# wgurecky/bipymc

Hardware: AMD Instinct MI355X
Metric: chain-updates/sec (higher is better)
Workload: dtype f64

## Files before the change

### bipymc_amd/csrc/kernels.h

```cpp
#pragma once
#ifndef __HIPCC_RTC__
#include <hip/hip_runtime.h>
#include <stdint.h>
#endif

#include "philox.h"

#ifdef BPM_STAMPS
#define BPM_STAMP(i)                                                                          \
    do {                                                                                      \
        __builtin_amdgcn_sched_barrier(0);                                                    \
        unsigned long long _t;                                                                \
        asm volatile("s_memtime %0\n\ts_waitcnt lgkmcnt(0)" : "=s"(_t)::"memory");            \
        __builtin_amdgcn_sched_barrier(0);                                                    \
        bpm_stamp[i] = _t;                                                                    \
    } while (0)
#else
#define BPM_STAMP(i) do { } while (0)
#endif

#if defined(__HIP_DEVICE_COMPILE__) && !defined(__gfx942__) && !defined(__gfx950__)
#error "kernels.h: the ticket hand-overs rely on gfx942 / gfx950 memory behaviour (vmcnt counts stores; agent-scope atomics bypass the L2s): use __ATOMIC_RELEASE / __ATOMIC_ACQUIRE tickets on other targets"
#endif

// ... 114 lines not shown
    uint32_t upd_off, n_upd, pool_off, M;
    uint32_t mode;
    uint32_t n_items;
    uint32_t algo;
    uint32_t P, n_cr;
    double* cr_part1;
    const double* cr_fold_part;
    const double* cr_fold_tot;
    double* cr_fold_out;
    uint32_t cr_fold_nb;
    uint32_t cr_chunk0, cr_n1;
    uint32_t adapt_on;
    uint32_t cr_gate;
    uint32_t hist_len;
    double gamma_scale, gamma_demc, epsilon, u_epsilon, p_snooker;
#ifdef BPM_LEAN_LAST
    uint32_t lean, pad_lean;
#endif
};

#ifdef BPM_TEST_HOOKS
__host__ __device__ __forceinline__ int32_t* trace_i32_of(const PhaseArgs& a) { return a.trace_i32; }
__host__ __device__ __forceinline__ double* trace_f64_of(const PhaseArgs& a) { return a.trace_f64; }
__host__ __device__ __forceinline__ uint8_t* trace_mask_of(const PhaseArgs& a) { return a.trace_mask; }
__host__ __device__ __forceinline__ void trace_set(PhaseArgs& a, int32_t* i, double* f, uint8_t* m) { a.trace_i32 = i; a.trace_f64 = f; a.trace_mask = m; }
#else
__host__ __device__ constexpr int32_t* trace_i32_of(const PhaseArgs&) { return nullptr; }
__host__ __device__ constexpr double* trace_f64_of(const PhaseArgs&) { return nullptr; }
__host__ __device__ constexpr uint8_t* trace_mask_of(const PhaseArgs&) { return nullptr; }
__host__ __device__ __forceinline__ void trace_set(PhaseArgs&, int32_t*, double*, uint8_t*) {}
#endif

template <int CTRL>
__device__ __forceinline__ double dpp_f64(double v) {
    const int lo = __builtin_amdgcn_update_dpp(0, __double2loint(v), CTRL, 0xF, 0xF, false);
    const int hi = __builtin_amdgcn_update_dpp(0, __double2hiint(v), CTRL, 0xF, 0xF, false);
    return __hiloint2double(hi, lo);
}
__device__ __forceinline__ double readlane_f64(double v, int lane) {
    return __hiloint2double(__builtin_amdgcn_readlane(__double2hiint(v), lane),
                            __builtin_amdgcn_readlane(__double2loint(v), lane));
}
template <int LPC>
__device__ __forceinline__ double gsum(double v) {
    static_assert(LPC == 1 || LPC == 4 || LPC == 16 || LPC == 32 || LPC == 64, "subgroup sizes");
    if (LPC >= 4) {
        v += dpp_f64<0xB1>(v);
        v += dpp_f64<0x4E>(v);
    }
    if (LPC >= 16) {
        v += dpp_f64<0x141>(v);
        v += dpp_f64<0x140>(v);
    }
    if (LPC == 32) v += __shfl_xor(v, 16);
    if (LPC == 64) v = (readlane_f64(v, 0) + readlane_f64(v, 16)) + (readlane_f64(v, 32) + readlane_f64(v, 48));
    return v;
}
template <int LPC>
__device__ __forceinline__ void gsum2(double& v, double& w) {
    static_assert(LPC == 1 || LPC == 4 || LPC == 16 || LPC == 32 || LPC == 64, "subgroup sizes");
    if (LPC >= 4) {
        const double v1 = dpp_f64<0xB1>(v), w1 = dpp_f64<0xB1>(w);
        v += v1; w += w1;
        const double v2 = dpp_f64<0x4E>(v), w2 = dpp_f64<0x4E>(w);
        v += v2; w += w2;
    }
    if (LPC >= 16) {
        const double v3 = dpp_f64<0x141>(v), w3 = dpp_f64<0x141>(w);
        v += v3; w += w3;
        const double v4 = dpp_f64<0x140>(v), w4 = dpp_f64<0x140>(w);
        v += v4; w += w4;
    }
    if (LPC == 32) { const double vs = __shfl_xor(v, 16), ws = __shfl_xor(w, 16); v += vs; w += ws; }
    if (LPC == 64) {
        const double va = readlane_f64(v, 0) + readlane_f64(v, 16), wa = readlane_f64(w, 0) + readlane_f64(w, 16);
        const double vb = readlane_f64(v, 32) + readlane_f64(v, 48), wb = readlane_f64(w, 32) + readlane_f64(w, 48);
        v = va + vb; w = wa + wb;
    }
}
template <int LPC>
__device__ __forceinline__ int gsum_i(int v) {
    if (LPC >= 4) {
        v += __builtin_amdgcn_update_dpp(0, v, 0xB1, 0xF, 0xF, false);
        v += __builtin_amdgcn_update_dpp(0, v, 0x4E, 0xF, 0xF, false);
    }
    if (LPC >= 16) {
        v += __builtin_amdgcn_update_dpp(0, v, 0x141, 0xF, 0xF, false);
        v += __builtin_amdgcn_update_dpp(0, v, 0x140, 0xF, 0xF, false);
    }
    if (LPC == 32) v += __shfl_xor(v, 16);
    if (LPC == 64)
        v = (__builtin_amdgcn_readlane(v, 0) + __builtin_amdgcn_readlane(v, 16)) +
            (__builtin_amdgcn_readlane(v, 32) + __builtin_amdgcn_readlane(v, 48));
    return v;
}

constexpr uint32_t CR_FINAL_MAX = 512;
__host__ __device__ inline uint32_t cr_chunks_of(uint32_t n_half, uint32_t g1) { return (n_half + g1 - 1u) / g1; }
struct CrTotals { double p[MAX_CR], d[MAX_CR], n[MAX_CR]; };
__device__ __forceinline__ void cr_finalize(bool any, uint32_t n_cr, CrTotals& T) {
    if (!any) return;
    uint32_t nz = 0;
#pragma unroll
    for (int m = 0; m < MAX_CR; ++m) nz += (m < (int)n_cr && T.n[m] != 0.0) ? 1u : 0u;
    if (nz == n_cr) {
#pragma unroll
        for (int m = 0; m < MAX_CR; ++m) if (m < (int)n_cr) T.p[m] = T.d[m] / T.n[m];
    }
    double sum = 0.0;
#pragma unroll
    for (int m = 0; m < MAX_CR; ++m) if (m < (int)n_cr) sum += T.p[m];
#pragma unroll
    for (int m = 0; m < MAX_CR; ++m) if (m < (int)n_cr) T.p[m] = T.p[m] / sum;
}
template <int ROUNDS>
__device__ __forceinline__ double cr_array_sum(const double* arr, uint32_t nb) {
    const uint32_t lane = threadIdx.x & (WAVE - 1);
    double v[ROUNDS];
#pragma unroll
    for (int r = 0; r < ROUNDS; ++r) {
        const uint32_t b = (uint32_t)r * WAVE + lane;
        const double x = arr[b < nb ? b : nb - 1u];
        v[r] = b < nb ? x : 0.0;
    }
    double s = 0.0;
#pragma unroll
// ... 224 lines not shown
__device__ __forceinline__ void store_row_sys(double* row, int q, uint32_t ld, const double* v) {
#pragma unroll
    for (int u = 0; u < DPL / 2; ++u) {
        const uint32_t pi = (uint32_t)(q + u * LPC);
        if (2 * pi < ld) {
            __hip_atomic_store(row + 2 * pi, v[2 * u], __ATOMIC_RELAXED, __HIP_MEMORY_SCOPE_SYSTEM);
            __hip_atomic_store(row + 2 * pi + 1, v[2 * u + 1], __ATOMIC_RELAXED, __HIP_MEMORY_SCOPE_SYSTEM);
        }
    }
}

template <int LPC, int DPL>
__device__ __forceinline__ void store_row_stream(double* row, int q, uint32_t ld, const double* v) {
#pragma unroll
    for (int u = 0; u < DPL / 2; ++u) {
        const uint32_t pi = (uint32_t)(q + u * LPC);
        if (2 * pi < ld) {
            bpm_d2v t = {v[2 * u], v[2 * u + 1]};
            __builtin_nontemporal_store(t, reinterpret_cast<bpm_d2v*>(row) + pi);
        }
    }
}

__device__ __forceinline__ void box_muller_pair_f32(uint32_t w1, uint32_t w2, double& n0, double& n1) {
    const float u1 = ((float)w1 + 1.0f) * 2.3283064365386963e-10f;
    const float u2 = (float)w2 * 2.3283064365386963e-10f;
    const float r = __builtin_amdgcn_sqrtf(-2.0f * 0.6931471805599453f * __builtin_amdgcn_logf(u1));
    n0 = (double)(r * __builtin_amdgcn_cosf(u2));
    n1 = (double)(r * __builtin_amdgcn_sinf(u2));
}

template <int K>
__device__ __forceinline__ uint32_t quad_bcast(uint32_t v) {
    return (uint32_t)__builtin_amdgcn_update_dpp(0, (int)v, K * 0x55, 0xF, 0xF, false);
}

template <int LPC, int NPART_CT>
struct Partners {
    uint32_t r[NPART_CT > 0 ? NPART_CT : 1];
    const uint32_t* lds;
    __device__ __forceinline__ uint32_t get(int i) const { return NPART_CT > 0 ? r[i] : lds[i]; }
};

__device__ __forceinline__ uint32_t partner_pos(const PhaseArgs& a, uint32_t c, uint32_t idx, uint32_t n_pair_idx) {
    if (idx < n_pair_idx) {
        const uint32_t p = idx >> 1;
        const u32x4 wb = chain_block(a.seed, c, a.t, SLOT_PAIR0 + (p >> 1));
        uint32_t ia, ib;
        distinct_pair((p & 1) ? wb.z : wb.x, (p & 1) ? wb.w : wb.y, a.M, ia, ib);
        uint32_t pos = (idx & 1) ? ib : ia;
        if (a.mode == 2) pos += (pos >= c) ? 1u : 0u;
        return pos;
    }
    const u32x4 ws = chain_block(a.seed, c, a.t, SLOT_SNK);
    uint32_t iz, i1, i2;
    distinct_three(ws.x, ws.y, ws.z, a.M, iz, i1, i2);
    const uint32_t s = idx - n_pair_idx;
    return s == 0 ? iz : (s == 1 ? i1 : i2);
}

__device__ __forceinline__ uint32_t pos_to_chain(const PhaseArgs& a, uint32_t pos) {
#if defined(BPM_TEST_HOOKS) && defined(BPM_FAKE_NO_PARTNER_HOP)
    return pos;
#else
    return a.perm_tab ? a.perm_tab[pos] : perm_fwd(pos, a.pk);
#endif
}
__device__ __forceinline__ uint32_t own_pos_to_chain(const PhaseArgs& a, uint32_t pos) {
#if defined(BPM_TEST_HOOKS) && defined(BPM_FAKE_NO_OWN_HOP)
    return pos;
#else
    return a.perm_tab ? a.perm_tab[pos] : perm_fwd(pos, a.pk);
#endif
}
__device__ __forceinline__ uint32_t chain_to_pos(const PhaseArgs& a, uint32_t c) {
    return a.inv_tab ? a.inv_tab[c] : perm_inv(c, a.pk);
}

template <int DPL, int NPX>
struct PlanFront {
    uint32_t rec[PLAN_WORDS];
    double x[DPL], ra[NPX][DPL], rb[NPX][DPL];
    double ll_cur, pcr[3], gl[DPL];
    uint32_t acc_prev;
};
typedef uint32_t bpm_u32x16 __attribute__((ext_vector_type(16)));
__device__ __forceinline__ bpm_u32x16 plan_record(const uint32_t* recp) {
    return *reinterpret_cast<const bpm_u32x16*>(__builtin_assume_aligned(recp, 4 * PLAN_WORDS));
}
template <int DPL, int NP>
__device__ __forceinline__ void plan_front(const Layout& L, const bpm_u32x16 rv, int q, PlanFront<DPL, (NP > 0 ? NP : 1)>& fr) {
    static_assert(PLAN_WORDS == 16 && DPL == 2, "one 64-byte record, one 16-byte load per lane and row");
#pragma unroll
    for (int i = 0; i < PLAN_WORDS; ++i) fr.rec[i] = rv[i];
    load_row_all<WAVE, DPL>(row_ptr(L, fr.rec[0]), q, L.ld, fr.x);
#pragma unroll
    for (int p = 0; p < NP; ++p) {
        load_row_all<WAVE, DPL>(row_ptr(L, fr.rec[5 + 2 * p]), q, L.ld, fr.ra[p]);
        load_row_all<WAVE, DPL>(row_ptr(L, fr.rec[5 + 2 * p + 1]), q, L.ld, fr.rb[p]);
    }
    __builtin_amdgcn_sched_barrier(0);
}

struct NoEarly { template <class W> __device__ __forceinline__ void operator()(W&) const {} };
struct PcrGiven { bool on = false; double p[MAX_CR]; };
template <int ALGO, int LPC, int DPL, int NP, int LOAD_LL = 1 , class EARLY = NoEarly, bool FRONT = false>
__device__ __forceinline__ void make_proposal(const PhaseArgs& a, uint32_t c, bool active, int q, int cw,
                                              uint32_t* s_part, Work<DPL>& wk, const uint32_t* rec = nullptr,
                                              unsigned long long* bpm_stamp = nullptr, EARLY early = EARLY(), const PcrGiven pcr_ovr = PcrGiven(),
                                              const PlanFront<DPL, (NP > 0 ? NP : 1)>* fr = nullptr) {
    static_assert(!FRONT || (LPC == WAVE && DPL == 2), "the planned front serves one wavefront per chain with one coordinate pair per lane");
    constexpr bool DREAM = ALGO == ALGO_DREAM;
    constexpr bool FAST = (NP > 0) && (LPC == 1);
    constexpr bool SNK_DIRECT = (LPC == 1);
    const uint32_t dim = a.L.dim, ld = a.L.ld;
    const uint32_t P = NP > 0 ? (uint32_t)NP : a.P;
    if constexpr (FRONT) {
        const bool in_row = 2u * (uint32_t)q < ld;
#pragma unroll
        for (int s = 0; s < DPL; ++s) wk.x[s] = in_row ? fr->x[s] : 0.0;
    } else
    load_row<LPC, DPL>(row_ptr(a.L, c), q, ld, wk.x);
    wk.ll_cur = 0.0;
    wk.acc_prev = 0u;
    if (!a.replay) {
#if defined(BPM_TEST_HOOKS) && defined(BPM_FAKE_NO_LL)
        if (LPC < WAVE) wk.ll_cur = wk.x[0] * 1e-300; else
#endif
        if constexpr (FRONT) wk.ll_cur = fr->ll_cur; else
        if (LOAD_LL == 1 || (LOAD_LL == 2 && !a.lean)) wk.ll_cur = a.ll[c - a.lo];
        if constexpr (FRONT) wk.acc_prev = fr->acc_prev; else
        if (LPC == WAVE) wk.acc_prev = a.acc_count[c - a.lo];
// ... 11 lines not shown
    double gtab[DPL];
    if (DREAM && LPC == WAVE) {
#pragma unroll
        for (int u = 0; u < DPL; ++u) {
            const uint32_t gi = (uint32_t)(q + u * WAVE);
            const double gl = FRONT ? fr->gl[u] : a.gamma_tab[gi <= dim ? gi : dim];
            gtab[u] = gi <= dim ? gl : 0.0;
        }
    }
    double gt_lane = 0.0;
    if (DREAM && LPC * DPL < WAVE) {
        const uint32_t wl = (uint32_t)threadIdx.x & (uint32_t)(WAVE - 1);
        gt_lane = a.gamma_tab[wl <= dim ? wl : dim];
    }
    const bool snk_possible = !DREAM && a.p_snooker > 0.0 && a.M >= 3;
    const uint32_t npart = 2 * P + (snk_possible ? 3u : 0u);
    constexpr bool RL = (LPC == WAVE) && (NP > 0) && !FAST;
    const uint32_t npairs = (dim + 1u) >> 1;
    const bool merged = !FRONT && RL && DPL == 2 && (npairs + 2u * (uint32_t)NP + 1u <= (uint32_t)WAVE);
    u32x4 wpair[DPL / 2];
    u32x4 h0;
    constexpr bool QUAD = DREAM && LPC == 4 && DPL == 2 && NP == 3;
    constexpr bool REGS = FAST || RL || QUAD;
    Partners<LPC, REGS ? 2 * NP : 0> part;
    part.lds = s_part + cw * MAX_PARTNERS;
    const bool planned = FRONT || ((LPC == WAVE) && rec != nullptr);
    const bool dims_late = planned && RL && DPL == 2;
    if (FRONT) {
        h0.x = fr->rec[1]; h0.y = fr->rec[2]; h0.z = fr->rec[3]; h0.w = fr->rec[4];
#pragma unroll
        for (int i = 0; i < 2 * NP; ++i) part.r[i] = fr->rec[5 + i];
        if (!dims_late) {
#pragma unroll
            for (int u = 0; u < DPL / 2; ++u) wpair[u] = chain_block(a.seed, c, a.t, SLOT_DIM0 + (uint32_t)(q + u * LPC));
        }
    } else if (planned) {
        h0.x = rec[1]; h0.y = rec[2]; h0.z = rec[3]; h0.w = rec[4];
        if (FAST || RL) {
#pragma unroll
            for (int i = 0; i < 2 * NP; ++i) part.r[i] = rec[5 + i];
        }
        if (!dims_late) {
#pragma unroll
            for (int u = 0; u < DPL / 2; ++u) wpair[u] = chain_block(a.seed, c, a.t, SLOT_DIM0 + (uint32_t)(q + u * LPC));
        }
    } else if (merged) {
        const uint32_t uq = (uint32_t)q, hdr_lane = npairs + 2u * (uint32_t)NP;
        const uint32_t pidx = uq - npairs;
        const uint32_t slot = uq < npairs ? SLOT_DIM0 + uq : (uq < hdr_lane ? SLOT_PAIR0 + (pidx >> 2) : SLOT_HDR0);
        const u32x4 wb = chain_block(a.seed, c, a.t, slot);
        wpair[0] = wb;
        h0.x = (uint32_t)__builtin_amdgcn_readlane((int)wb.x, hdr_lane);
        h0.y = (uint32_t)__builtin_amdgcn_readlane((int)wb.y, hdr_lane);
        h0.z = (uint32_t)__builtin_amdgcn_readlane((int)wb.z, hdr_lane);
        h0.w = (uint32_t)__builtin_amdgcn_readlane((int)wb.w, hdr_lane);
        BPM_STAMP(2);
        uint32_t mine = 0;
        if (uq >= npairs && uq < hdr_lane) {
            const uint32_t p = pidx >> 1;
            uint32_t ia, ib;
            distinct_pair((p & 1) ? wb.z : wb.x, (p & 1) ? wb.w : wb.y, a.M, ia, ib);
            uint32_t pos = (pidx & 1) ? ib : ia;
            if (a.mode == 2) pos += (pos >= c) ? 1u : 0u;
            mine = pos_to_chain(a, a.pool_off + pos);
        }
#pragma unroll
        for (int i = 0; i < 2 * NP; ++i) part.r[i] = (uint32_t)__builtin_amdgcn_readlane((int)mine, npairs + i);
    } else if (QUAD) {
        wpair[0] = chain_block(a.seed, c, a.t, SLOT_DIM0 + (uint32_t)q);
        const u32x4 wb = chain_block(a.seed, c, a.t, q == 1 ? SLOT_PAIR0 : (q == 2 ? SLOT_PAIR0 + 1u : SLOT_HDR0));
        h0.x = quad_bcast<0>(wb.x); h0.y = quad_bcast<0>(wb.y); h0.z = quad_bcast<0>(wb.z); h0.w = quad_bcast<0>(wb.w);
        uint32_t i0 = 0, i1 = 0, i2 = 0, i3 = 0;
        if (q == 1 || q == 2) {
            uint32_t ia, ib;
            distinct_pair(wb.x, wb.y, a.M, ia, ib);
            i0 = pos_to_chain(a, a.pool_off + ia); i1 = pos_to_chain(a, a.pool_off + ib);
            if (q == 1) {
                distinct_pair(wb.z, wb.w, a.M, ia, ib);
                i2 = pos_to_chain(a, a.pool_off + ia); i3 = pos_to_chain(a, a.pool_off + ib);
            }
        }
        part.r[0] = quad_bcast<1>(i0); part.r[1] = quad_bcast<1>(i1); part.r[2] = quad_bcast<1>(i2); part.r[3] = quad_bcast<1>(i3);
        part.r[4] = quad_bcast<2>(i0); part.r[5] = quad_bcast<2>(i1);
    } else {
        h0 = chain_block(a.seed, c, a.t, SLOT_HDR0);
#pragma unroll
        for (int u = 0; u < DPL / 2; ++u) wpair[u] = chain_block(a.seed, c, a.t, SLOT_DIM0 + (uint32_t)(q + u * LPC));
        if (FAST) {
#pragma unroll
            for (int i = 0; i < 2 * NP; ++i) part.r[i] = pos_to_chain(a, a.pool_off + partner_pos(a, c, (uint32_t)i, 2u * NP));
        }
        if (RL) {
            uint32_t mine = 0;
            if (q < 2 * NP) mine = pos_to_chain(a, a.pool_off + partner_pos(a, c, (uint32_t)q, 2u * NP));
#pragma unroll
            for (int i = 0; i < 2 * NP; ++i) part.r[i] = (uint32_t)__builtin_amdgcn_readlane((int)mine, i);
        }
    }
    BPM_STAMP(3);
    wk.u_acc = u01_53(h0.z, h0.w);
    const double u_sel = (double)(h0.x >> 16) * 1.52587890625e-05;
    const double u_gam = (double)(h0.x & 0xFFFFu) * 1.52587890625e-05;
    uint32_t snk_id[3] = {0u, 0u, 0u};
    if (SNK_DIRECT && snk_possible && planned) {
        snk_id[0] = rec[5 + 2 * P]; snk_id[1] = rec[6 + 2 * P]; snk_id[2] = rec[7 + 2 * P];
    } else if (SNK_DIRECT && snk_possible && (u_sel < a.p_snooker || trace_i32_of(a) != nullptr)) {
        const u32x4 ws = chain_block(a.seed, c, a.t, SLOT_SNK);
        uint32_t iz, i1, i2;
        distinct_three(ws.x, ws.y, ws.z, a.M, iz, i1, i2);
        snk_id[0] = pos_to_chain(a, a.pool_off + iz);
        snk_id[1] = pos_to_chain(a, a.pool_off + i1);
        snk_id[2] = pos_to_chain(a, a.pool_off + i2);
    }
    if (!REGS || (snk_possible && !SNK_DIRECT)) {
#pragma unroll 1
        for (uint32_t idx = (uint32_t)q; idx < npart; idx += LPC)
            s_part[cw * MAX_PARTNERS + idx] = planned ? rec[5 + idx] : pos_to_chain(a, a.pool_off + partner_pos(a, c, idx, 2 * P));
        __builtin_amdgcn_fence(__ATOMIC_RELEASE, "wavefront");
        __builtin_amdgcn_wave_barrier();
        __builtin_amdgcn_fence(__ATOMIC_ACQUIRE, "wavefront");
    }

    constexpr int NPX = NP > 0 ? NP : 1;
    double ra[NPX][DPL], rb[NPX][DPL];
    if (FRONT && DREAM && NP > 0) {
#pragma unroll
        for (int p = 0; p < NP; ++p) {
#pragma unroll
            for (int s = 0; s < DPL; ++s) { ra[p][s] = fr->ra[p][s]; rb[p][s] = fr->rb[p][s]; }
        }
    } else if (DREAM && NP > 0) {
#pragma unroll
        for (int p = 0; p < NP; ++p) {
            if (LPC == WAVE) {
                load_row_all<LPC, DPL>(row_ptr(a.L, part.get(2 * p)), q, ld, ra[p]);
                load_row_all<LPC, DPL>(row_ptr(a.L, part.get(2 * p + 1)), q, ld, rb[p]);
            } else {
                load_row<LPC, DPL>(row_ptr(a.L, part.get(2 * p)), q, ld, ra[p]);
                load_row<LPC, DPL>(row_ptr(a.L, part.get(2 * p + 1)), q, ld, rb[p]);
            }
        }
    }
    if (!FRONT) BPM_STAMP(7);
    if (dims_late) wpair[0] = chain_block(a.seed, c, a.t, SLOT_DIM0 + (uint32_t)q);
    if (DREAM) early(wk);

    double eps_n[DPL], eps_u[DPL];
    uint32_t maskbits = 0;
    wk.cr_idx = -1; wk.d_prime = (int)dim; wk.jump = 0; wk.snk = 0; wk.delta = 0.0; wk.log_corr = 0.0;
    uint32_t thr = 65536u;
    if (DREAM) {
        const double uc = u_sel;
        double cum = 0.0;
        int idx = (int)a.n_cr - 1;
        bool found = false;
#pragma unroll
        for (int m = 0; m < MAX_CR; ++m) {
            if (m < (int)a.n_cr) {
                cum += pcr[m];
                if (!found && uc < cum) { idx = m; thr = a.thr[m]; found = true; }
            }
        }
        if (!found) {
#pragma unroll
            for (int m = 0; m < MAX_CR; ++m) if (m == (int)a.n_cr - 1) thr = a.thr[m];
        }
        wk.cr_idx = idx;
    }
    int cnt = 0;
#pragma unroll
    for (int u = 0; u < DPL / 2; ++u) {
        const uint32_t pi = (uint32_t)(q + u * LPC);
        const uint32_t j0 = 2u * pi;
        eps_n[2 * u] = 0.0; eps_n[2 * u + 1] = 0.0; eps_u[2 * u] = 0.0; eps_u[2 * u + 1] = 0.0;
        if (j0 < dim) {
            const u32x4 wj = wpair[u];
            const bool two = j0 + 1 < dim;
// ... 720 lines not shown
    const int cw = lane / LPC, q = lane % LPC;
    const uint32_t w = blockIdx.x * (block_for(LPC) / LPC) + cw;
    bool active = w < a.n_items;
    int32_t id = active ? a.ids_buf[w] : -1;
    active = active && id >= 0;
    if (LPC == WAVE && !active) return;
    const uint32_t c = active ? (uint32_t)id : a.lo;
    Work<DPL> wk;
    load_row<LPC, DPL>(row_ptr(a.L, c), q, a.L.ld, wk.x);
    load_row<LPC, DPL>(a.prop_buf + (uint64_t)(active ? w : 0u) * a.L.ld, q, a.L.ld, wk.p);
    wk.log_corr = active ? a.aux_buf[w] : 0.0;
    wk.ll_cur = a.ll[c - a.lo];
    wk.acc_prev = a.acc_count[c - a.lo];
    if (ALGO == ALGO_DREAM && a.adapt_on) {
        load_row<LPC, DPL>(a.w_mean + (uint32_t)((c - a.lo) * 2u * a.L.ld), q, a.L.ld, wk.w_mean);
        load_row<LPC, DPL>(a.w_m2 + (uint32_t)((c - a.lo) * 2u * a.L.ld), q, a.L.ld, wk.w_m2);
    }
    const double ll_prop = active ? a.aux_buf[a.L.n_local + w] : 0.0;
    const u32x4 h0 = chain_block(a.seed, c, a.t, SLOT_HDR0);
    wk.u_acc = u01_53(h0.z, h0.w);
    wk.delta = 0.0; wk.gamma = 0.0; wk.cr_idx = -1; wk.d_prime = 0; wk.jump = 0; wk.snk = 0; wk.maskbits = 0; wk.item = w; wk.pos_own = 0u;
    if (ALGO == ALGO_DREAM && active) {
        wk.delta = *delta_ptr(a.L, c);
        wk.cr_idx = (int)*cridx_ptr(a.L, c);
    }
    PhaseArgs b = a;
    if (ALGO == ALGO_DREAM) b.cr_gate = (wk.cr_idx >= 0) ? 1u : 0u;
    finish_update<ALGO, LPC, DPL>(b, c, active, q, wk, ll_prop);
}

constexpr int CR_L1_THREADS = 256;
template <int G1, int J>
__device__ __forceinline__ int cr_bcast_i(int v) {
    if (G1 == 4) return __builtin_amdgcn_update_dpp(0, v, J * 0x55, 0xF, 0xF, false);
    if (G1 == 16) return __builtin_amdgcn_update_dpp(0, v, 0x150 + J, 0xF, 0xF, false);
    return __builtin_amdgcn_readlane(v, J);
}
template <int G1, int J>
__device__ __forceinline__ void cr_l1_steps(int idx, double dl, int m0, double& sd0, double& sn0, double& sd1, double& sn1) {
    const int ij = cr_bcast_i<G1, J>(idx);
    const double dj = __hiloint2double(cr_bcast_i<G1, J>(__double2hiint(dl)), cr_bcast_i<G1, J>(__double2loint(dl)));
    cr_chunk_add(sd0, sn0, m0, ij, dj);
    if (G1 == 4) cr_chunk_add(sd1, sn1, m0 + 4, ij, dj);
    if constexpr (J + 1 < G1) cr_l1_steps<G1, J + 1>(idx, dl, m0, sd0, sn0, sd1, sn1);
}
template <int G1>
__global__ __launch_bounds__(CR_L1_THREADS) void cr_level1_kernel(Layout L, PermKey pk, const uint32_t* perm_tab, uint32_t N, uint32_t n_cr, uint32_t n1, double* part1) {
    const uint32_t t = blockIdx.x * CR_L1_THREADS + threadIdx.x;
    const uint32_t ch = t / G1, k = t % G1;
    const uint32_t n_first = (N + 1u) / 2u, c_first = cr_chunks_of(n_first, G1);
    const bool second = ch >= c_first;
    const uint32_t pos = second ? n_first + (ch - c_first) * G1 + k : ch * G1 + k;
    const bool valid = ch < n1 && pos < (second ? N : n_first);
    int idx = -1;
    double dl = 0.0;
    if (valid) {
        const uint32_t c = perm_tab ? perm_tab[pos] : perm_fwd(pos, pk);
        idx = (int)*cridx_ptr(L, c);
        dl = *delta_ptr(L, c);
    }
    static_assert(MAX_CR <= 8, "a chunk's lanes cover the CR values: lane k sums value k (and k + 4 when G1 == 4)");
    double sd0 = 0.0, sn0 = 0.0, sd1 = 0.0, sn1 = 0.0;
    cr_l1_steps<G1, 0>(idx, dl, (int)k, sd0, sn0, sd1, sn1);
    if (ch < n1) {
        if (k < n_cr) {
            __hip_atomic_store(&part1[(uint64_t)k * n1 + ch], sd0, __ATOMIC_RELAXED, __HIP_MEMORY_SCOPE_AGENT);
            __hip_atomic_store(&part1[(uint64_t)(MAX_CR + k) * n1 + ch], sn0, __ATOMIC_RELAXED, __HIP_MEMORY_SCOPE_AGENT);
        }
// ... 740 lines not shown
```

### bipymc_amd/csrc/kernels_wide.h

```cpp
#pragma once
#include "kernels.h"

namespace bpm {
inline namespace BPM_VARIANT_NS {

constexpr int WIDE_CP = 2;
constexpr int WIDE_CHUNK_PAIRS = WAVE * WIDE_CP;

template <int TARGET>
struct WideTarget {
    __device__ __forceinline__ void add(const double*, uint32_t, uint32_t, double, double) {}
    __device__ __forceinline__ double finish(const double*, uint32_t) { return 0.0; }
};
template <>
struct WideTarget<TARGET_GAUSS> {
    double s1 = 0.0, s2 = 0.0;
    __device__ __forceinline__ void add(const double* tp, uint32_t pi, uint32_t dim, double v0, double v1) {
        const uint32_t j0 = 2u * pi;
        if (j0 < dim) {
            const double2 is = *reinterpret_cast<const double2*>(tp + 4 + j0);
            const double z0 = v0 * is.x;
            s1 += z0; s2 += z0 * z0;
            if (j0 + 1u < dim) {
                const double z1 = v1 * is.y;
// ... 30 lines not shown
        return m + log(exp(c0 - m) + exp(c1 - m));
    }
};

__device__ __forceinline__ double2 wide_load2(const double* row, uint32_t pi, bool valid) {
    double2 t = make_double2(0.0, 0.0);
    if (valid) t = reinterpret_cast<const double2*>(row)[pi];
    return t;
}
__device__ __forceinline__ void wide_store2_stream(double* row, uint32_t pi, double v0, double v1) {
    bpm_d2v t = {v0, v1};
    __builtin_nontemporal_store(t, reinterpret_cast<bpm_d2v*>(row) + pi);
}
__device__ __forceinline__ void wide_store2_wt16(double* row, uint32_t pi, double v0, double v1) {
    bpm_d2v t = {v0, v1};
    bpm_d2v* p = reinterpret_cast<bpm_d2v*>(row) + pi;
    asm volatile("global_store_dwordx4 %0, %1, off sc1" ::"v"(p), "v"(t) : "memory");
}

struct WideUni {
    uint32_t dim, ld, P;
    uint32_t thr, forced;
    double gamma;
    double epsilon, u_epsilon;
    int snk;
    double gs;
};
template <int ALGO, int NP>
__device__ __forceinline__ void wide_pair_proposal(const PhaseArgs& a, const WideUni& U, uint32_t c, uint32_t pi, bool valid, double2 x, uint32_t mine,
                                                   double& p0, double& p1, uint32_t& mbits) {
    constexpr bool DREAM = ALGO == ALGO_DREAM;
    const uint32_t j0 = 2u * pi;
    const bool two = j0 + 1u < U.dim;
    const u32x4 wj = chain_block(a.seed, c, a.t, SLOT_DIM0 + pi);
    double en0 = 0.0, en1 = 0.0, eu0 = 0.0, eu1 = 0.0;
    mbits = 0u;
    if (valid) {
        if (U.epsilon > 0.0) {
            double n0, n1;
            box_muller_pair_f32(wj.z, wj.w, n0, n1);
            en0 = U.epsilon * n0;
            if (two) en1 = U.epsilon * n1;
        }
        if (DREAM) {
            if (U.u_epsilon > 0.0) {
                eu0 = -U.u_epsilon + (2.0 * U.u_epsilon) * (((double)(wj.y >> 16) + 0.5) * 1.52587890625e-05);
                if (two) eu1 = -U.u_epsilon + (2.0 * U.u_epsilon) * (((double)(wj.y & 0xFFFFu) + 0.5) * 1.52587890625e-05);
            }
            if ((wj.x >> 16) <= U.thr || j0 == U.forced) mbits |= 1u;
            if (two && ((wj.x & 0xFFFFu) <= U.thr || j0 + 1u == U.forced)) mbits |= 2u;
        }
    }
    if (DREAM) {
        double s0 = 0.0, s1 = 0.0;
        if (NP > 0) {
            double2 ra[NP > 0 ? NP : 1], rb[NP > 0 ? NP : 1];
#pragma unroll
            for (int p = 0; p < NP; ++p) {
                ra[p] = wide_load2(row_ptr(a.L, (uint32_t)__builtin_amdgcn_readlane((int)mine, 2 * p)), pi, valid);
                rb[p] = wide_load2(row_ptr(a.L, (uint32_t)__builtin_amdgcn_readlane((int)mine, 2 * p + 1)), pi, valid);
            }
            s0 = ra[0].x - rb[0].x; s1 = ra[0].y - rb[0].y;
#pragma unroll
            for (int p = 1; p < NP; ++p) { s0 = s0 + (ra[p].x - rb[p].x); s1 = s1 + (ra[p].y - rb[p].y); }
        } else {
#pragma unroll 1
            for (uint32_t p = 0; p < U.P; ++p) {
// ... 62 lines not shown
    uint32_t mine = 0;
    if (lane < npart) mine = pos_to_chain(a, a.pool_off + partner_pos(a, c, lane, 2u * U.P));
    double ll_cur = 0.0;
    uint32_t acc_prev = 0u;
    if (FUSED) { ll_cur = a.ll[li]; acc_prev = a.acc_count[li]; }
    const double u_sel = (double)(h0.x >> 16) * 1.52587890625e-05;
    const double u_gam = (double)(h0.x & 0xFFFFu) * 1.52587890625e-05;
    int cr_idx = -1, d_prime = (int)U.dim, jump = 0;
    if (DREAM) {
        double cum = 0.0;
        int idx = (int)a.n_cr - 1;
        bool found = false;
#pragma unroll
        for (int m = 0; m < MAX_CR; ++m) {
            if (m < (int)a.n_cr) {
                cum += a.cr_state[m];
                if (!found && u_sel < cum) { idx = m; found = true; }
            }
        }
        cr_idx = idx;
#pragma unroll
        for (int m = 0; m < MAX_CR; ++m) if (m == idx) U.thr = a.thr[m];
        int cnt = (int)U.dim;
        if (U.thr < 65536u) {
            cnt = 0;
#pragma unroll 1
            for (uint32_t k = 0; k < n_chunks; ++k) {
#pragma unroll
                for (int u = 0; u < WIDE_CP; ++u) {
                    const uint32_t pi = k * WIDE_CHUNK_PAIRS + (uint32_t)u * WAVE + lane;
                    const uint32_t j0 = 2u * pi;
                    bool b0 = false, b1 = false;
                    if (j0 < U.dim) {
                        const u32x4 wj = chain_block(a.seed, c, a.t, SLOT_DIM0 + pi);
                        b0 = (wj.x >> 16) <= U.thr;
                        b1 = (j0 + 1u < U.dim) && (wj.x & 0xFFFFu) <= U.thr;
                    }
                    cnt += (int)__popcll(__ballot(b0)) + (int)__popcll(__ballot(b1));
                }
            }
        }
        if (cnt == 0) { U.forced = mulhi32(h0.y, U.dim); cnt = 1; }
        d_prime = cnt;
        double gamma = a.gamma_tab[cnt];
        if (a.k % 5 == 0 && !(u_gam < 0.2)) { gamma = 1.0; jump = 1; }
        U.gamma = gamma;
    } else {
        double gamma = a.gamma_demc;
        if (a.mode != 2 && a.k % 10 == 0 && !(u_gam < 0.1)) { gamma = 1.0; jump = 1; }
        U.gamma = gamma;
    }
    double sn_n2 = 0.0;
    if (snk_possible && u_sel < a.p_snooker) {
        const double* zrow = row_ptr(a.L, (uint32_t)__builtin_amdgcn_readlane((int)mine, 2));
        const double* r1row = row_ptr(a.L, (uint32_t)__builtin_amdgcn_readlane((int)mine, 3));
        const double* r2row = row_ptr(a.L, (uint32_t)__builtin_amdgcn_readlane((int)mine, 4));
        double n2 = 0.0, dot = 0.0;
#pragma unroll 1
        for (uint32_t k = 0; k < n_chunks; ++k) {
#pragma unroll
            for (int u = 0; u < WIDE_CP; ++u) {
                const uint32_t pi = k * WIDE_CHUNK_PAIRS + (uint32_t)u * WAVE + lane;
                const bool valid = 2u * pi < U.dim;
                const double2 x = wide_load2(xrow, pi, valid), z = wide_load2(zrow, pi, valid), r1 = wide_load2(r1row, pi, valid), r2 = wide_load2(r2row, pi, valid);
                const double d0 = x.x - z.x, d1 = x.y - z.y;
                n2 += d0 * d0; dot += (r1.x - r2.x) * d0;
                n2 += d1 * d1; dot += (r1.y - r2.y) * d1;
// ... 247 lines not shown
```

### bipymc_amd/csrc/philox.h

```cpp
#pragma once
#ifndef __HIPCC_RTC__
#include <stdint.h>
#endif

#if defined(__HIPCC__)
#define BPM_HD __host__ __device__ __forceinline__
#else
#define BPM_HD inline
#endif

#ifndef BPM_VARIANT_NS
#ifdef BPM_TEST_HOOKS
#define BPM_VARIANT_NS hooks
#else
#define BPM_VARIANT_NS product
#endif
#endif
namespace bpm {
inline namespace BPM_VARIANT_NS {

constexpr int SLOT_BITS = 16;
constexpr uint32_t SLOT_HDR0 = 0;
constexpr uint32_t SLOT_PAIR0 = 2;
constexpr uint32_t SLOT_SNK = 7;
constexpr uint32_t SLOT_DIM0 = 8;
constexpr int MAX_PAIRS = 10;
constexpr uint64_t SUBSEQ_GLOBAL = 0xFFFFFFFFFFFFFFFFull;
constexpr uint32_t SLOT_G_FLIP = 0;
constexpr uint32_t SLOT_G_SHUF = 1;
constexpr uint64_t T_INIT = (1ull << 47) - 1;
constexpr int FEISTEL_ROUNDS = 6;

struct u32x4 {
    uint32_t x, y, z, w;
};

BPM_HD uint32_t mulhi32(uint32_t a, uint32_t b) {
#if defined(__HIP_DEVICE_COMPILE__)
    return __umulhi(a, b);
#else
    return (uint32_t)(((uint64_t)a * (uint64_t)b) >> 32);
#endif
}

BPM_HD u32x4 philox4x32_10(uint32_t c0, uint32_t c1, uint32_t c2, uint32_t c3, uint32_t k0, uint32_t k1) {
    constexpr uint32_t M0 = 0xD2511F53u, M1 = 0xCD9E8D57u, W0 = 0x9E3779B9u, W1 = 0xBB67AE85u;
#pragma unroll
    for (int r = 0; r < 10; ++r) {
        const uint64_t p0 = (uint64_t)M0 * (uint64_t)c0, p1 = (uint64_t)M1 * (uint64_t)c2;
        const uint32_t hi0 = (uint32_t)(p0 >> 32), lo0 = (uint32_t)p0;
        const uint32_t hi1 = (uint32_t)(p1 >> 32), lo1 = (uint32_t)p1;
        const uint32_t n0 = hi1 ^ c1 ^ k0, n2 = hi0 ^ c3 ^ k1;
        c0 = n0; c1 = lo1; c2 = n2; c3 = lo0;
        k0 += W0; k1 += W1;
    }
    return u32x4{c0, c1, c2, c3};
}

BPM_HD u32x4 philox_block(uint64_t seed, uint64_t subseq, uint64_t blk) {
    return philox4x32_10((uint32_t)blk, (uint32_t)(blk >> 32), (uint32_t)subseq, (uint32_t)(subseq >> 32),
                         (uint32_t)seed, (uint32_t)(seed >> 32));
}

BPM_HD u32x4 chain_block(uint64_t seed, uint64_t chain_id, uint64_t t, uint32_t slot) {
#if defined(BPM_TEST_HOOKS) && defined(BPM_FAKE_DRAWS) && defined(__HIP_DEVICE_COMPILE__)
    uint32_t x = (uint32_t)chain_id * 0x9e3779b9u + (uint32_t)t * 0x85ebca6bu + slot * 0xc2b2ae35u + (uint32_t)seed;
    x ^= x >> 15; x *= 0x2c1b3c6du; x ^= x >> 12;
    return u32x4{x, x * 0x297a2d39u, x ^ 0x5bd1e995u, x + 0x7f4a7c15u};
#else
    return philox_block(seed, chain_id, (t << SLOT_BITS) | (uint64_t)slot);
#endif
}

BPM_HD u32x4 global_block(uint64_t seed, uint64_t t, uint32_t slot) {
    return chain_block(seed, SUBSEQ_GLOBAL, t, slot);
}

BPM_HD double u01_32(uint32_t w) { return (double)w * 2.3283064365386963e-10; }

BPM_HD double u01_53(uint32_t hi, uint32_t lo) {
    return ((double)(hi >> 5) * 67108864.0 + (double)(lo >> 6)) * 1.1102230246251565e-16;
}

BPM_HD void distinct_pair(uint32_t wa, uint32_t wb, uint32_t m, uint32_t& ia, uint32_t& ib) {
    ia = mulhi32(wa, m);
    ib = mulhi32(wb, m - 1);
    ib += (ib >= ia) ? 1u : 0u;
}

BPM_HD void distinct_three(uint32_t wz, uint32_t w1, uint32_t w2, uint32_t m, uint32_t& iz, uint32_t& i1,
                           uint32_t& i2) {
    iz = mulhi32(wz, m);
    i1 = mulhi32(w1, m - 1);
    i1 += (i1 >= iz) ? 1u : 0u;
    const uint32_t lo = iz < i1 ? iz : i1, hi = iz < i1 ? i1 : iz;
    i2 = mulhi32(w2, m - 2);
    i2 += (i2 >= lo) ? 1u : 0u;
    i2 += (i2 >= hi) ? 1u : 0u;
}

BPM_HD uint32_t hash32(uint32_t x) {
    x ^= x >> 16; x *= 0x7FEB352Du; x ^= x >> 15; x *= 0x846CA68Bu; x ^= x >> 16;
    return x;
// ... 75 lines not shown
```

Measured before the change: 790.5 million.

## Use row-broadcast DPP reductions, bitop3 Philox XOR, and pinned scalar row bases

Several independent micro-optimisations land together. Full-wave sums now use DPP row_bcast15/31 followed by a single readlane instead of four readlanes, and DPP moves use mov_dpp with bound_ctrl. Philox rounds called from per-lane contexts use the gfx950 bitop3 three-input XOR to cut VALU instructions. The plan-front row loads precompute the base pointers, pin them in SGPRs through empty asm, and issue one clamped 16-byte global load per row in place of the generic load helper. The clamped index and changed reduction order can alter rounding and edge behaviour.

Measured after the change: 827.2 million, median of 6. +4.6%, better.

```diff
diff --git a/bipymc_amd/csrc/kernels.h b/bipymc_amd/csrc/kernels.h
--- a/bipymc_amd/csrc/kernels.h
+++ b/bipymc_amd/csrc/kernels.h
@@ -170,14 +170,24 @@
 #endif
 
 template <int CTRL>
+__device__ __forceinline__ int dpp_i32(int v) {
+    return __builtin_amdgcn_mov_dpp(v, CTRL, 0xF, 0xF, true);
+}
+template <int CTRL>
 __device__ __forceinline__ double dpp_f64(double v) {
-    const int lo = __builtin_amdgcn_update_dpp(0, __double2loint(v), CTRL, 0xF, 0xF, false);
-    const int hi = __builtin_amdgcn_update_dpp(0, __double2hiint(v), CTRL, 0xF, 0xF, false);
+    const int lo = dpp_i32<CTRL>(__double2loint(v));
+    const int hi = dpp_i32<CTRL>(__double2hiint(v));
     return __hiloint2double(hi, lo);
 }
 __device__ __forceinline__ double readlane_f64(double v, int lane) {
     return __hiloint2double(__builtin_amdgcn_readlane(__double2hiint(v), lane),
                             __builtin_amdgcn_readlane(__double2loint(v), lane));
+}
+constexpr int DPP_ROW_BCAST15 = 0x142, DPP_ROW_BCAST31 = 0x143;
+__device__ __forceinline__ double row_sums_step1_f64(double v) { return v + dpp_f64<DPP_ROW_BCAST15>(v); }
+__device__ __forceinline__ double row_sums_step2_f64(double v) { return v + dpp_f64<DPP_ROW_BCAST31>(v); }
+__device__ __forceinline__ double row_sums_f64(double v) {
+    return readlane_f64(row_sums_step2_f64(row_sums_step1_f64(v)), WAVE - 1);
 }
 template <int LPC>
 __device__ __forceinline__ double gsum(double v) {
@@ -191,7 +201,7 @@
         v += dpp_f64<0x140>(v);
     }
     if (LPC == 32) v += __shfl_xor(v, 16);
-    if (LPC == 64) v = (readlane_f64(v, 0) + readlane_f64(v, 16)) + (readlane_f64(v, 32) + readlane_f64(v, 48));
+    if (LPC == 64) v = row_sums_f64(v);
     return v;
 }
 template <int LPC>
@@ -211,25 +221,27 @@
     }
     if (LPC == 32) { const double vs = __shfl_xor(v, 16), ws = __shfl_xor(w, 16); v += vs; w += ws; }
     if (LPC == 64) {
-        const double va = readlane_f64(v, 0) + readlane_f64(v, 16), wa = readlane_f64(w, 0) + readlane_f64(w, 16);
-        const double vb = readlane_f64(v, 32) + readlane_f64(v, 48), wb = readlane_f64(w, 32) + readlane_f64(w, 48);
-        v = va + vb; w = wa + wb;
+        v = row_sums_step1_f64(v); w = row_sums_step1_f64(w);
+        v = row_sums_step2_f64(v); w = row_sums_step2_f64(w);
+        v = readlane_f64(v, WAVE - 1); w = readlane_f64(w, WAVE - 1);
     }
 }
 template <int LPC>
 __device__ __forceinline__ int gsum_i(int v) {
     if (LPC >= 4) {
-        v += __builtin_amdgcn_update_dpp(0, v, 0xB1, 0xF, 0xF, false);
-        v += __builtin_amdgcn_update_dpp(0, v, 0x4E, 0xF, 0xF, false);
+        v += dpp_i32<0xB1>(v);
+        v += dpp_i32<0x4E>(v);
     }
     if (LPC >= 16) {
-        v += __builtin_amdgcn_update_dpp(0, v, 0x141, 0xF, 0xF, false);
-        v += __builtin_amdgcn_update_dpp(0, v, 0x140, 0xF, 0xF, false);
+        v += dpp_i32<0x141>(v);
+        v += dpp_i32<0x140>(v);
     }
     if (LPC == 32) v += __shfl_xor(v, 16);
-    if (LPC == 64)
-        v = (__builtin_amdgcn_readlane(v, 0) + __builtin_amdgcn_readlane(v, 16)) +
-            (__builtin_amdgcn_readlane(v, 32) + __builtin_amdgcn_readlane(v, 48));
+    if (LPC == 64) {
+        v += dpp_i32<DPP_ROW_BCAST15>(v);
+        v += dpp_i32<DPP_ROW_BCAST31>(v);
+        v = __builtin_amdgcn_readlane(v, WAVE - 1);
+    }
     return v;
 }
 
@@ -520,7 +532,7 @@
 
 template <int K>
 __device__ __forceinline__ uint32_t quad_bcast(uint32_t v) {
-    return (uint32_t)__builtin_amdgcn_update_dpp(0, (int)v, K * 0x55, 0xF, 0xF, false);
+    return (uint32_t)dpp_i32<K * 0x55>((int)v);
 }
 
 template <int LPC, int NPART_CT>
@@ -581,11 +593,24 @@
     static_assert(PLAN_WORDS == 16 && DPL == 2, "one 64-byte record, one 16-byte load per lane and row");
 #pragma unroll
     for (int i = 0; i < PLAN_WORDS; ++i) fr.rec[i] = rv[i];
-    load_row_all<WAVE, DPL>(row_ptr(L, fr.rec[0]), q, L.ld, fr.x);
+    typedef const __attribute__((address_space(1))) bpm_d2v* grow_t;
+    const double* base[1 + 2 * (NP > 0 ? NP : 1)];
+    base[0] = row_ptr(L, fr.rec[0]);
+#pragma unroll
+    for (int i = 0; i < 2 * NP; ++i) base[1 + i] = row_ptr(L, fr.rec[5 + i]);
+#ifndef BPM_STAMPS
+#pragma unroll
+    for (int i = 0; i < 1 + 2 * NP; ++i) asm("" : "+s"(base[i]));
+#endif
+    const uint32_t last = (L.ld >> 1) - 1u, pi = (uint32_t)q < last ? (uint32_t)q : last;
+    bpm_d2v t = ((grow_t)base[0])[pi];
+    fr.x[0] = t.x; fr.x[1] = t.y;
 #pragma unroll
     for (int p = 0; p < NP; ++p) {
-        load_row_all<WAVE, DPL>(row_ptr(L, fr.rec[5 + 2 * p]), q, L.ld, fr.ra[p]);
-        load_row_all<WAVE, DPL>(row_ptr(L, fr.rec[5 + 2 * p + 1]), q, L.ld, fr.rb[p]);
+        t = ((grow_t)base[1 + 2 * p])[pi];
+        fr.ra[p][0] = t.x; fr.ra[p][1] = t.y;
+        t = ((grow_t)base[2 + 2 * p])[pi];
+        fr.rb[p][0] = t.x; fr.rb[p][1] = t.y;
     }
     __builtin_amdgcn_sched_barrier(0);
 }
@@ -663,7 +688,7 @@
         for (int i = 0; i < 2 * NP; ++i) part.r[i] = fr->rec[5 + i];
         if (!dims_late) {
 #pragma unroll
-            for (int u = 0; u < DPL / 2; ++u) wpair[u] = chain_block(a.seed, c, a.t, SLOT_DIM0 + (uint32_t)(q + u * LPC));
+            for (int u = 0; u < DPL / 2; ++u) wpair[u] = chain_block<true>(a.seed, c, a.t, SLOT_DIM0 + (uint32_t)(q + u * LPC));
         }
     } else if (planned) {
         h0.x = rec[1]; h0.y = rec[2]; h0.z = rec[3]; h0.w = rec[4];
@@ -673,13 +698,13 @@
         }
         if (!dims_late) {
 #pragma unroll
-            for (int u = 0; u < DPL / 2; ++u) wpair[u] = chain_block(a.seed, c, a.t, SLOT_DIM0 + (uint32_t)(q + u * LPC));
+            for (int u = 0; u < DPL / 2; ++u) wpair[u] = chain_block<true>(a.seed, c, a.t, SLOT_DIM0 + (uint32_t)(q + u * LPC));
         }
     } else if (merged) {
         const uint32_t uq = (uint32_t)q, hdr_lane = npairs + 2u * (uint32_t)NP;
         const uint32_t pidx = uq - npairs;
         const uint32_t slot = uq < npairs ? SLOT_DIM0 + uq : (uq < hdr_lane ? SLOT_PAIR0 + (pidx >> 2) : SLOT_HDR0);
-        const u32x4 wb = chain_block(a.seed, c, a.t, slot);
+        const u32x4 wb = chain_block<true>(a.seed, c, a.t, slot);
         wpair[0] = wb;
         h0.x = (uint32_t)__builtin_amdgcn_readlane((int)wb.x, hdr_lane);
         h0.y = (uint32_t)__builtin_amdgcn_readlane((int)wb.y, hdr_lane);
@@ -698,8 +723,8 @@
 #pragma unroll
         for (int i = 0; i < 2 * NP; ++i) part.r[i] = (uint32_t)__builtin_amdgcn_readlane((int)mine, npairs + i);
     } else if (QUAD) {
-        wpair[0] = chain_block(a.seed, c, a.t, SLOT_DIM0 + (uint32_t)q);
-        const u32x4 wb = chain_block(a.seed, c, a.t, q == 1 ? SLOT_PAIR0 : (q == 2 ? SLOT_PAIR0 + 1u : SLOT_HDR0));
+        wpair[0] = chain_block<true>(a.seed, c, a.t, SLOT_DIM0 + (uint32_t)q);
+        const u32x4 wb = chain_block<true>(a.seed, c, a.t, q == 1 ? SLOT_PAIR0 : (q == 2 ? SLOT_PAIR0 + 1u : SLOT_HDR0));
         h0.x = quad_bcast<0>(wb.x); h0.y = quad_bcast<0>(wb.y); h0.z = quad_bcast<0>(wb.z); h0.w = quad_bcast<0>(wb.w);
         uint32_t i0 = 0, i1 = 0, i2 = 0, i3 = 0;
         if (q == 1 || q == 2) {
@@ -714,9 +739,9 @@
         part.r[0] = quad_bcast<1>(i0); part.r[1] = quad_bcast<1>(i1); part.r[2] = quad_bcast<1>(i2); part.r[3] = quad_bcast<1>(i3);
         part.r[4] = quad_bcast<2>(i0); part.r[5] = quad_bcast<2>(i1);
     } else {
-        h0 = chain_block(a.seed, c, a.t, SLOT_HDR0);
-#pragma unroll
-        for (int u = 0; u < DPL / 2; ++u) wpair[u] = chain_block(a.seed, c, a.t, SLOT_DIM0 + (uint32_t)(q + u * LPC));
+        h0 = chain_block<(LPC < WAVE)>(a.seed, c, a.t, SLOT_HDR0);
+#pragma unroll
+        for (int u = 0; u < DPL / 2; ++u) wpair[u] = chain_block<true>(a.seed, c, a.t, SLOT_DIM0 + (uint32_t)(q + u * LPC));
         if (FAST) {
 #pragma unroll
             for (int i = 0; i < 2 * NP; ++i) part.r[i] = pos_to_chain(a, a.pool_off + partner_pos(a, c, (uint32_t)i, 2u * NP));
@@ -773,7 +798,7 @@
         }
     }
     if (!FRONT) BPM_STAMP(7);
-    if (dims_late) wpair[0] = chain_block(a.seed, c, a.t, SLOT_DIM0 + (uint32_t)q);
+    if (dims_late) wpair[0] = chain_block<true>(a.seed, c, a.t, SLOT_DIM0 + (uint32_t)q);
     if (DREAM) early(wk);
 
     double eps_n[DPL], eps_u[DPL];
@@ -1560,8 +1585,8 @@
 constexpr int CR_L1_THREADS = 256;
 template <int G1, int J>
 __device__ __forceinline__ int cr_bcast_i(int v) {
-    if (G1 == 4) return __builtin_amdgcn_update_dpp(0, v, J * 0x55, 0xF, 0xF, false);
-    if (G1 == 16) return __builtin_amdgcn_update_dpp(0, v, 0x150 + J, 0xF, 0xF, false);
+    if (G1 == 4) return dpp_i32<J * 0x55>(v);
+    if (G1 == 16) return dpp_i32<0x150 + J>(v);
     return __builtin_amdgcn_readlane(v, J);
 }
 template <int G1, int J>
diff --git a/bipymc_amd/csrc/kernels_wide.h b/bipymc_amd/csrc/kernels_wide.h
--- a/bipymc_amd/csrc/kernels_wide.h
+++ b/bipymc_amd/csrc/kernels_wide.h
@@ -86,7 +86,7 @@
     constexpr bool DREAM = ALGO == ALGO_DREAM;
     const uint32_t j0 = 2u * pi;
     const bool two = j0 + 1u < U.dim;
-    const u32x4 wj = chain_block(a.seed, c, a.t, SLOT_DIM0 + pi);
+    const u32x4 wj = chain_block<true>(a.seed, c, a.t, SLOT_DIM0 + pi);
     double en0 = 0.0, en1 = 0.0, eu0 = 0.0, eu1 = 0.0;
     mbits = 0u;
     if (valid) {
@@ -215,7 +215,7 @@
                     const uint32_t j0 = 2u * pi;
                     bool b0 = false, b1 = false;
                     if (j0 < U.dim) {
-                        const u32x4 wj = chain_block(a.seed, c, a.t, SLOT_DIM0 + pi);
+                        const u32x4 wj = chain_block<true>(a.seed, c, a.t, SLOT_DIM0 + pi);
                         b0 = (wj.x >> 16) <= U.thr;
                         b1 = (j0 + 1u < U.dim) && (wj.x & 0xFFFFu) <= U.thr;
                     }
diff --git a/bipymc_amd/csrc/philox.h b/bipymc_amd/csrc/philox.h
--- a/bipymc_amd/csrc/philox.h
+++ b/bipymc_amd/csrc/philox.h
@@ -43,32 +43,50 @@
 #endif
 }
 
-BPM_HD u32x4 philox4x32_10(uint32_t c0, uint32_t c1, uint32_t c2, uint32_t c3, uint32_t k0, uint32_t k1) {
+BPM_HD uint32_t xor3(uint32_t a, uint32_t b, uint32_t c) {
+#if defined(__HIP_DEVICE_COMPILE__) && defined(__gfx950__) && defined(__has_builtin)
+#if __has_builtin(__builtin_amdgcn_bitop3_b32)
+    return __builtin_amdgcn_bitop3_b32(a, b, c, 0x96);
+#else
+    return a ^ b ^ c;
+#endif
+#else
+    return a ^ b ^ c;
+#endif
+}
+
+template <bool LANES>
+BPM_HD u32x4 philox4x32_10_t(uint32_t c0, uint32_t c1, uint32_t c2, uint32_t c3, uint32_t k0, uint32_t k1) {
     constexpr uint32_t M0 = 0xD2511F53u, M1 = 0xCD9E8D57u, W0 = 0x9E3779B9u, W1 = 0xBB67AE85u;
 #pragma unroll
     for (int r = 0; r < 10; ++r) {
         const uint64_t p0 = (uint64_t)M0 * (uint64_t)c0, p1 = (uint64_t)M1 * (uint64_t)c2;
         const uint32_t hi0 = (uint32_t)(p0 >> 32), lo0 = (uint32_t)p0;
         const uint32_t hi1 = (uint32_t)(p1 >> 32), lo1 = (uint32_t)p1;
-        const uint32_t n0 = hi1 ^ c1 ^ k0, n2 = hi0 ^ c3 ^ k1;
+        const uint32_t n0 = (LANES && r >= 2) ? xor3(hi1, c1, k0) : (hi1 ^ c1 ^ k0), n2 = (LANES && r >= 2) ? xor3(hi0, c3, k1) : (hi0 ^ c3 ^ k1);
         c0 = n0; c1 = lo1; c2 = n2; c3 = lo0;
         k0 += W0; k1 += W1;
     }
     return u32x4{c0, c1, c2, c3};
 }
-
-BPM_HD u32x4 philox_block(uint64_t seed, uint64_t subseq, uint64_t blk) {
-    return philox4x32_10((uint32_t)blk, (uint32_t)(blk >> 32), (uint32_t)subseq, (uint32_t)(subseq >> 32),
-                         (uint32_t)seed, (uint32_t)(seed >> 32));
+BPM_HD u32x4 philox4x32_10(uint32_t c0, uint32_t c1, uint32_t c2, uint32_t c3, uint32_t k0, uint32_t k1) {
+    return philox4x32_10_t<false>(c0, c1, c2, c3, k0, k1);
 }
 
+template <bool LANES = false>
+BPM_HD u32x4 philox_block(uint64_t seed, uint64_t subseq, uint64_t blk) {
+    return philox4x32_10_t<LANES>((uint32_t)blk, (uint32_t)(blk >> 32), (uint32_t)subseq, (uint32_t)(subseq >> 32),
+                                  (uint32_t)seed, (uint32_t)(seed >> 32));
+}
+
+template <bool LANES = false>
 BPM_HD u32x4 chain_block(uint64_t seed, uint64_t chain_id, uint64_t t, uint32_t slot) {
 #if defined(BPM_TEST_HOOKS) && defined(BPM_FAKE_DRAWS) && defined(__HIP_DEVICE_COMPILE__)
     uint32_t x = (uint32_t)chain_id * 0x9e3779b9u + (uint32_t)t * 0x85ebca6bu + slot * 0xc2b2ae35u + (uint32_t)seed;
     x ^= x >> 15; x *= 0x2c1b3c6du; x ^= x >> 12;
     return u32x4{x, x * 0x297a2d39u, x ^ 0x5bd1e995u, x + 0x7f4a7c15u};
 #else
-    return philox_block(seed, chain_id, (t << SLOT_BITS) | (uint64_t)slot);
+    return philox_block<LANES>(seed, chain_id, (t << SLOT_BITS) | (uint64_t)slot);
 #endif
 }
 
```
